# Zeudon/sound-event-localization-detection

Measured on AMD Instinct MI355X. Metric: training clips/sec (4ch FOA 60s@24kHz), higher is better.
Workload: dtype bf16; 1 GPU; crnn FOA 4-ch 60s clips, bs=32 windows (BASELINE configs[1]); parallelism=dp1

## Files before the change

include/seld_hip.h:

```cpp
#ifndef SELD_HIP_H_
#define SELD_HIP_H_

#include <stdint.h>

#ifdef __cplusplus
extern "C" {
#endif

int seld_init(int device);
int seld_shutdown(void);
int seld_version(void);
const char* seld_last_error(void);

int seld_set_mel_filterbank(const float* fb_host);

int seld_set_window(const float* window_host);

int seld_default_tables(float* window960, float* fb481x64, int* mel_b0_64, float* mel_wd_24x64,
                        float* mel_wu_24x64);

int64_t seld_num_frames(int64_t L);

int seld_logmel_f32(const float* pcm, int64_t N, int64_t C, int64_t L, float* out, int layout, void* stream);
int seld_logmel_i16(const int16_t* pcm, int64_t N, int64_t C, int64_t L, float* out, int layout, void* stream);
// ... 100 lines not shown
int64_t seld_softmax_mse_workspace_bytes(void);
int seld_softmax_mse(const void* logits, int logits_is_bf16, const uint16_t* mask, const float* dense_labels,
                     int64_t n_cells, int num_classes, float grad_scale, float* loss_out, void* grad,
                     void* workspace, void* stream);

int64_t seld_softmax_ce_workspace_bytes(void);
int seld_softmax_ce(const void* logits, int logits_is_bf16, const uint16_t* mask, const float* dense_labels,
                    int64_t n_cells, int num_classes, const float* class_weights, float focal_gamma, float grad_scale,
                    float* out, void* grad, void* workspace, void* stream);

int seld_scale_by_device_scalar(void* data, int is_bf16, int64_t n, const float* scale, void* stream);

int seld_multi_adam(const void* const* grad, const int32_t* grad_is_bf16, float* const* param, float* const* exp_avg,
                    float* const* exp_avg_sq, void* const* low_bf16, const int64_t* lengths, int count, const float* lr,
                    const float* step, float beta1, float beta2, float eps, float weight_decay, float grad_scale,
                    void* stream);

typedef struct seld_guard_record {
  float grad_norm;
  float clip_coef;
  float apply;
  float skipped;
  int32_t steps_skipped;
  int32_t steps_clipped;
  int32_t reserved[2];
} seld_guard_record;

int seld_multi_grad_norm_scratch(const int64_t* lengths, int count, int64_t* partial_floats);
int seld_multi_grad_norm(const void* const* grad, const int32_t* grad_is_bf16, const int64_t* lengths, int count,
                         float grad_scale, float max_norm, int skip_nonfinite, float* partial, int64_t partial_floats,
                         seld_guard_record* guard, void* stream);

int seld_multi_adam_guarded(const void* const* grad, const int32_t* grad_is_bf16, float* const* param,
                            float* const* exp_avg, float* const* exp_avg_sq, void* const* low_bf16, const int64_t* lengths,
                            int count, const float* lr, const float* step, float beta1, float beta2, float eps,
                            float weight_decay, float grad_scale, float* const* ema, float ema_decay,
                            const seld_guard_record* guard, void* stream);

int seld_multi_cast(const void* const* src, void* const* dst, const int64_t* lengths, int count, int bf16_to_fp32,
                    void* stream);

int seld_layernorm_supported(int64_t D);
int64_t seld_layernorm_workspace_floats(int64_t rows, int64_t D);
int seld_layernorm_forward(const void* x, int is_bf16, int64_t rows, int64_t D, const float* weight, const float* bias,
                           float eps, int relu, void* y, float* mean_rstd, void* stream);
int seld_layernorm_backward(const void* x, const void* dy, int is_bf16, int64_t rows, int64_t D, const float* weight,
                            const float* bias, const float* mean_rstd, int relu, void* dx, float* dweight,
                            float* dbias, float* workspace, void* stream);

int seld_stream_delay(int64_t nanoseconds, void* stream);

int64_t seld_smr_loss_workspace_bytes(int64_t frames, int64_t cells_per_frame);
int seld_smr_loss(const void* logits, int logits_is_bf16, const uint16_t* mask, const float* dense_labels,
                  int64_t frames, int rows, int cols, int num_classes, float w_class, float w_aiur, float w_cl,
                  float* loss_out4, void* grad, void* workspace, void* stream);


int seld_gru_fold_bias(const float* b_ih, const float* b_hh, int64_t H, void* gi_bias, int out_is_bf16, float* b_hn,
                       void* stream);

int seld_gru_prepare(const float* b_ih, const float* b_hh, const void* w_hh, int w_is_bf16, int64_t H, void* gi_bias,
                     int out_is_bf16, float* b_hn, void* w_hh_t_bf16, void* stream);

int seld_gru_bias_grads(const float* partial, int64_t tiles, int64_t H, float* db_ih, float* db_hh, void* stream);

int seld_sum_chunks(const void* partial, int in_is_bf16, int64_t chunks, int64_t count, void* out, int out_is_bf16,
                    void* stream);

int seld_sum_chunks_columns(const void* partial, int in_is_bf16, int64_t chunks, int64_t rows, int64_t C, int64_t F,
                            void* out, int out_is_bf16, void* stream);

int64_t seld_column_sums_blocks(int64_t rows, int64_t n_cols);
int seld_column_sums(const void* g, int in_is_bf16, int64_t rows, int64_t n_cols, float* partial, void* out, int out_is_bf16,
                     void* stream);

int seld_multi_sum_chunks(const void* const* partial, void* const* out, const int64_t* counts, const int32_t* chunks,
                          const int32_t* flags, int count, void* stream);
int seld_multi_column_sums_scratch(const int64_t* rows, const int64_t* n_cols, int count, int64_t* partial_floats);
int seld_multi_column_sums(const void* const* g, void* const* out, const int64_t* rows, const int64_t* n_cols,
                           const int32_t* flags, int count, float* partial, int64_t partial_floats, void* stream);

int seld_gru_dwhh_finish(const void* p_gi, const void* p_n, int in_is_bf16, int64_t chunks, int64_t H, void* dw_hh,
                         int out_is_bf16, void* stream);

int seld_conv_weight_flip_transpose(const void* w, int elem_bytes, int64_t O, int64_t I, void* wt, void* stream);

int seld_conv3x3_wgrad_supported(int64_t F, int64_t Cin, int64_t Cout);
int64_t seld_conv3x3_wgrad_workspace_floats(int64_t B, int64_t T, int64_t F, int64_t Cin, int64_t Cout);
int seld_conv3x3_wgrad(const void* x, const void* dy, int64_t B, int64_t T, int64_t F, int64_t Cin, int64_t Cout,
                       void* dw, int dw_is_bf16, float* workspace, void* stream);

int seld_conv3x3_dgrad_supported(int64_t F, int64_t Cin, int64_t Cout);
int seld_conv3x3_dgrad(const void* dy, const void* w, int64_t B, int64_t T, int64_t F, int64_t Cin, int64_t Cout,
                       void* dx, void* stream);

int seld_conv3x3_forward_supported(int64_t F, int64_t Cin, int64_t Cout);
int64_t seld_conv3x3_forward_chunks(int64_t B, int64_t T, int64_t F);
int seld_conv3x3_forward(const void* x, const void* w, int64_t B, int64_t T, int64_t F, int64_t Cin, int64_t Cout,
                         void* y, float* partials, void* stream);

int seld_convfirst_supported(int64_t F, int64_t Cin, int64_t Cout);
int64_t seld_convfirst_workspace_floats(int backward);
int seld_convfirst_forward(const void* in, const void* w, int w_is_bf16, int64_t w_sco, int64_t w_sci, int64_t w_sr,
                           int64_t w_ss, int64_t B, int64_t T, int64_t F, const float* bn_weight, const float* bn_bias,
                           float* running_mean, float* running_var, float momentum, float eps, void* y,
                           float* mean_invstd, float* scale_shift, float* workspace, int phases, void* stream);
int seld_convfirst_backward(const void* in, const void* w, int w_is_bf16, int64_t w_sco, int64_t w_sci, int64_t w_sr,
                            int64_t w_ss, const void* dy, int64_t B, int64_t T, int64_t F, const float* mean_invstd,
                            const float* scale_shift, void* dw, int dw_is_bf16, int64_t dw_sco, int64_t dw_sci,
                            int64_t dw_sr, int64_t dw_ss, float* dgamma, float* dbeta, float* workspace, int phases,
                            void* stream);

int64_t seld_conv_tail_workspace_floats(int C);
int seld_conv_tail_forward(const void* x, const void* residual, int is_bf16, int64_t rows, int C, int pool,
                           const float* weight, const float* bias, float* running_mean, float* running_var,
                           float momentum, float eps, int training, void* y, float* mean_invstd, float* scale_shift,
                           float* workspace, void* stream);
int64_t seld_conv_tail_partial_rows(void);
int seld_conv_tail_forward_from_partials(const void* x, int is_bf16, int64_t rows, int C, int pool,
                                         const float* partials, int64_t nrows, const float* weight, const float* bias,
                                         float* running_mean, float* running_var, float momentum, float eps, void* y,
                                         float* mean_invstd, float* scale_shift, void* stream);
int seld_conv_tail_backward(const void* x, const void* residual, const void* dy, int is_bf16, int64_t rows, int C,
                            int pool, const float* mean_invstd, const float* scale_shift, void* dx, void* dresidual,
                            float* dweight, float* dbias, float* workspace, void* stream);

int seld_dwconv1d(const void* x, int is_bf16, const float* weight, const float* bias, int64_t B, int64_t T, int D, int K,
                  int flip_taps, void* y, void* stream);
int64_t seld_dwconv1d_wgrad_rows(int64_t B, int64_t T);
int seld_dwconv1d_wgrad(const void* x, const void* dy, int is_bf16, int64_t B, int64_t T, int D, int K, float* partial,
                        void* stream);

int64_t seld_gru_tile_rows(void);
int seld_gru_forward(const void* gi, int is_bf16, const void* w_hh_bf16, const float* b_hn, int64_t B,
                     int64_t T, int64_t H, void* y, void* saved_tile, void* stream);

int seld_gru_backward(const void* dy_tile, const void* saved_tile, const void* y, int is_bf16,
                      const void* w_hh_t_bf16, int64_t tiles, int64_t T, int64_t H, void* dg_tile, float* dbias,
                      void* stream);

int seld_gru_backward_direct(const void* dy, const void* saved_tile, const void* y, int is_bf16,
                             const void* w_hh_t_bf16, int64_t B, int64_t T, int64_t H, void* dgi, void* dghn,
                             float* dbias, void* stream);

int seld_gru_to_tile(const void* src, int elem_bytes, int64_t B, int64_t T, int ns, void* dst, void* stream);
int seld_gru_from_pair_tile(const void* dg_tile, int elem_bytes, int64_t B, int64_t T, void* dgi, void* dghn,
                            void* stream);

int seld_gru_previous_state(const void* y, int elem_bytes, int64_t B, int64_t T, void* h_prev, void* stream);

int seld_grid_decode(const void* logits, int is_bf16, int64_t w0, int64_t nw, int64_t W, int64_t total,
                     const int64_t* meta_first, const int32_t* meta_len, int64_t q0, int64_t nq, float threshold, int K,
                     int32_t* det_cell, float* det_score, int32_t* det_count, float* probs_out, void* stream);

int seld_doa_match(const int32_t* det_cell, const int32_t* det_count, int K, const int32_t* ref_offsets,
                   const int32_t* ref_dirs, int64_t nq, int I, int J, double thr_deg, int32_t* stats, double* cost,
                   void* stream);

int seld_grid_decode_tta(const void* logits, int is_bf16, int64_t w0, int64_t nw, int64_t W, int64_t total,
                         const int64_t* meta_first, const int32_t* meta_len, int64_t q0, int64_t nq,
                         const int32_t* patterns, int n_patterns, float threshold, int K, int32_t* det_cell,
                         float* det_score, int32_t* det_count, float* probs_out, void* stream);

int seld_track_link(const int32_t* det_cell, const int32_t* det_count, int K, const int64_t* seg_offsets, int64_t S,
                    const int32_t* dist_table, int I, int J, int gate_mdeg, int max_gap, int min_len,
                    const int64_t* chain_offsets, int32_t* trk_cell, int32_t* trk_id, int32_t* trk_count, int32_t* tracks,
// ... 44 lines not shown
```

sound-event-localization-detection_amd/seld_gru.py:

```python
import torch
import torch.nn.functional as F

import seld_native
import seld_overlap
from seld_linear import chunk_count, tall_chunks, tall_product

HIDDEN = 256
direct_backward = True


def applicable(module, x):
    low = torch.is_autocast_enabled() or x.dtype in (torch.bfloat16, torch.float16)
    if not low and not getattr(module, "allow_fp32", False):
        return False
    return (module.hidden_size == HIDDEN and module.bidirectional and module.batch_first and module.bias
            and x.dim() == 3 and x.dtype in (torch.float32, torch.bfloat16, torch.float16) and module.proj_size == 0)


class _BiGRULayer(torch.autograd.Function):
    @staticmethod
    def forward(ctx, x, w_ih, b_ih, w_hh, b_hh, overlap=False, feature_cf=None):
        ctx.overlap = overlap
        ctx.feature_cf = feature_cf
        if feature_cf is not None:
            c, f = feature_cf
            w_ih = w_ih.view(w_ih.shape[0], c, f).transpose(1, 2).reshape(w_ih.shape[0], f * c)
        low = torch.is_autocast_enabled() or x.dtype == torch.bfloat16
        cdt = torch.bfloat16 if low else torch.float32
        with torch.autocast(device_type="cuda", enabled=False):
            xc = x.to(cdt)
            need = x.requires_grad or w_ih.requires_grad or w_hh.requires_grad
            w_hh_t = None
            if b_ih.dtype == torch.float32 and b_hh.dtype == torch.float32 and b_ih.is_contiguous() and b_hh.is_contiguous():
                if (direct_backward and need and w_hh.is_contiguous()
                        and w_hh.dtype in (torch.float32, torch.bfloat16)):
                    gi_bias, b_hn, w_hh_t = seld_native.gru_prepare(b_ih, b_hh.reshape(-1), w_hh, cdt)
                else:
                    gi_bias, b_hn = seld_native.gru_fold_bias(b_ih, b_hh.reshape(-1), cdt)
            else:
                fold = b_hh.clone()
                fold[:, 2 * HIDDEN:] = 0
                gi_bias, b_hn = (b_ih + fold.reshape(-1)).to(cdt), b_hh[:, 2 * HIDDEN:]
            gi = F.linear(xc, w_ih.to(cdt), gi_bias)
            b, t, _ = gi.shape
            y, saved = seld_native.gru_forward(gi.view(b, t, 2, 3 * HIDDEN), w_hh, b_hn, need)
        ctx.save_for_backward(xc, w_ih, w_hh, y, saved if saved is not None else torch.empty(0),
                              w_hh_t if w_hh_t is not None else torch.empty(0))
        ctx.cdt = cdt
        ctx.dtypes = (w_ih.dtype, b_ih.dtype, w_hh.dtype, b_hh.dtype)
        return y

    @staticmethod
    def backward(ctx, dy):
        xc, w_ih, w_hh, y, saved, w_hh_t = ctx.saved_tensors
        cdt = ctx.cdt
        b, t, _ = y.shape
        h = HIDDEN
        n = b * t
        with torch.autocast(device_type="cuda", enabled=False):
            dyc = dy.to(y.dtype)
            seld_overlap.launch_pending(dy.device)
            dgi, dghn, dbias = seld_native.gru_backward(dyc, saved, y, w_hh, raw_bias=True,
                                                        w_hh_t=w_hh_t if w_hh_t.numel() else None, direct=direct_backward)
            dgi2 = dgi.view(n, 6 * h)
            x2 = xc.reshape(n, -1)
            t_wih, t_bih, t_whh, t_bhh = ctx.dtypes

            dw_ih = torch.empty((6 * h, x2.shape[1]), dtype=t_wih, device=dy.device)
            dw_hh = torch.empty((2, 3 * h, h), dtype=t_whh, device=dy.device)
            db_ih = torch.empty(6 * h, dtype=t_bih, device=dy.device)
            db_hh = torch.empty(6 * h, dtype=t_bhh, device=dy.device)

            def weight_grads():
                fp32 = [db if db.dtype == torch.float32 else torch.empty(6 * h, dtype=torch.float32, device=dy.device)
                        for db in (db_ih, db_hh)]
                seld_native.gru_bias_grads(dbias, out=fp32)
                for db, full in zip((db_ih, db_hh), fp32):
                    if db is not full:
                        db.copy_(full)
                tall_product(dgi2, x2, out=dw_ih, columns_cf=ctx.feature_cf)
                hp = seld_native.gru_previous_state(y).view(n, 2 * h)
                chunks = chunk_count(n, 6 * h, 2 * h)
                p_gi = tall_chunks(dgi2, hp, chunks)
                p_n = tall_chunks(dghn.view(n, 2 * h), hp, chunks)
                seld_native.gru_dwhh_finish(p_gi, p_n, dw_hh)

            dx = (dgi2 @ w_ih.to(cdt)).view_as(xc)
            if ctx.overlap:
                seld_overlap.submit(dy.device, [dgi, dghn, y, xc, dbias, dw_ih, dw_hh, db_ih, db_hh], weight_grads)
            elif seld_overlap.conv_wgrad_side and seld_overlap.enabled and dy.is_cuda:
                seld_overlap.launch_now(dy.device, [dgi, dghn, y, xc, dbias, dw_ih, dw_hh, db_ih, db_hh], weight_grads,
                                        last_of_stage=True, outputs=[dw_ih, dw_hh, db_ih, db_hh])
            else:
                weight_grads()
        return dx.to(dy.dtype) if dx.dtype != dy.dtype and not torch.is_autocast_enabled() else dx, \
            dw_ih.view_as(dw_ih), db_ih.view_as(db_ih), dw_hh.view_as(dw_hh), db_hh.view(2, 3 * h), None, None


from seld_pack import adjacent as _adjacent, join as _join, pack as _pack


def pack_parameters(module):
    with torch.no_grad():
        for layer in range(module.num_layers):
            for kind in ("weight_ih", "bias_ih", "weight_hh", "bias_hh"):
                _pack((getattr(module, f"{kind}_l{layer}"), getattr(module, f"{kind}_l{layer}_reverse")))


def bigru_forward(module, x, feature_cf=None, overlap=False, need_hn=True):
    overlap = overlap and seld_overlap.active(x)
    params = []
    for layer in range(module.num_layers):
        p = lambda name: getattr(module, f"{name}_l{layer}")
        pr = lambda name: getattr(module, f"{name}_l{layer}_reverse")
        group = (_join(p("weight_ih"), pr("weight_ih")), _join(p("bias_ih"), pr("bias_ih")),
                 _join(p("weight_hh"), pr("weight_hh")), _join(p("bias_hh"), pr("bias_hh")))
        params.append(seld_overlap.defer(*group) if overlap and layer > 0 else group)
    out = x
    finals = []
    for layer in range(module.num_layers):
        w_ih, b_ih, w_hh, b_hh = params[layer]
        out = _BiGRULayer.apply(out, w_ih, b_ih, w_hh.view(2, 3 * HIDDEN, HIDDEN), b_hh.view(2, 3 * HIDDEN),
                                overlap and layer > 0, feature_cf if layer == 0 else None)
        if need_hn:
            finals += [out[:, -1, :HIDDEN], out[:, 0, HIDDEN:]]
        if module.training and module.dropout > 0 and layer + 1 < module.num_layers:
            out = F.dropout(out, p=module.dropout, training=True)
    return out, (torch.stack(finals, dim=0) if need_hn else None)
```

sound-event-localization-detection_amd/seld_native.py:

```python
from __future__ import annotations

import ctypes
import os
import threading
from pathlib import Path

import torch

from seld_augment import PARAM_INTS as AUGMENT_PARAM_INTS, PATTERNS as AUGMENT_PATTERNS, check_channel_order

_HERE = Path(__file__).resolve().parent
LIB_PATH = Path(os.environ["SELD_HIP_LIB"]).resolve() if os.environ.get("SELD_HIP_LIB") else _HERE / "libseld_hip.so"

N_FFT = 960
HOP = 480
N_BINS = 481
N_MELS = 64

_lock = threading.Lock()
_lib = None
_initialised_devices = set()

_i64 = ctypes.c_int64
_int = ctypes.c_int
# ... 15 lines not shown
    lib.seld_default_tables.argtypes = [_ptr] * 5
    lib.seld_num_frames.restype = _i64
    lib.seld_num_frames.argtypes = [_i64]
    for name in ("seld_logmel_f32", "seld_logmel_i16"):
        getattr(lib, name).argtypes = [_ptr, _i64, _i64, _i64, _ptr, _int, _ptr]
    for name in ("seld_logmel_f32_strided", "seld_logmel_i16_strided"):
        getattr(lib, name).argtypes = [_ptr, _i64, _i64, _i64, _ptr, _i64, _i64, _i64, _i64, _ptr]
    for name in ("seld_stft_f32", "seld_stft_i16"):
        getattr(lib, name).argtypes = [_ptr, _i64, _i64, _i64, _ptr, _ptr]
    lib.seld_foa_intensity.argtypes = [_ptr, _i64, _i64, _ptr, _i64, _i64, _i64, _i64, _ptr]
    for fn in (lib.seld_logmel_iv_f32, lib.seld_logmel_iv_i16):
        fn.argtypes = [_ptr, _i64, _i64, _ptr, _i64, _i64, _i64, _i64, _ptr]
    for fn in (lib.seld_logmel_spectrum_f32, lib.seld_logmel_spectrum_i16):
        fn.argtypes = [_ptr, _i64, _i64, _i64, _ptr, _i64, _i64, _i64, _i64, _ptr, _ptr]
        fn.restype = ctypes.c_int
    for fn in (lib.seld_logmel_phasors_f32, lib.seld_logmel_phasors_i16):
        fn.argtypes = [_ptr, _i64, _i64, _i64, _ptr, _i64, _i64, _i64, _i64, _ptr, _ptr]
    lib.seld_phasor_pitch.restype = ctypes.c_int64
    lib.seld_gcc_phat_q15.argtypes = [_ptr, _i64, _i64, _i64, _ptr, _i64, _i64, _i64, _i64, _ptr]
    lib.seld_gcc_table_host.argtypes = [_ptr]
    lib.seld_gcc_phat.argtypes = [_ptr, _i64, _i64, _i64, _ptr, _i64, _i64, _i64, _i64, _ptr]
    lib.seld_nipd_table_host.argtypes = [ctypes.c_double, ctypes.c_double, ctypes.c_double, _ptr, _ptr, _ptr, _ptr]
    lib.seld_nipd_table_bytes.restype = _i64
    lib.seld_nipd_table_bytes.argtypes = []
    lib.seld_nipd_q15.argtypes = [_ptr, _i64, _i64, _i64, _ptr, _ptr, _i64, _i64, _i64, _i64, _ptr]
    lib.seld_labels_rasterise.argtypes = [_ptr, _i64, _i64, _int, _int, _ptr, _ptr]
    lib.seld_labels_expand.argtypes = [_ptr, _i64, _int, _ptr, _ptr]
    lib.seld_labels_rasterise_box.argtypes = [_ptr, _ptr, _i64, _i64, _int, _int, ctypes.c_double, ctypes.c_double, _ptr,
                                              _ptr]
    lib.seld_window_gather.argtypes = [_ptr, _i64, _i64, _ptr, _i64, _i64, _ptr, _ptr]
    lib.seld_window_gather_augment.argtypes = [_ptr, _i64, _int, _int, _ptr, _ptr, _i64, _i64, _ptr, ctypes.c_float, _ptr, _ptr]
    lib.seld_window_permute_mask.argtypes = [_ptr, _i64, _int, _int, _ptr, _ptr, _i64, _i64, _ptr, _ptr]
    lib.seld_foa_rotation_terms.argtypes = [_ptr, _i64, _i64, _int, _int, _ptr, _i64, _i64, _i64, _i64, _ptr]
    lib.seld_window_gather_rotate.argtypes = [_ptr, _ptr, _i64, _int, _int, _int, _int, _int, _int, _ptr, _ptr, _i64, _i64, _ptr,
                                              ctypes.c_float, _ptr, _ptr]
    lib.seld_window_permute_mask_rotate.argtypes = [_ptr, _i64, _int, _int, _ptr, _ptr, _i64, _i64, _ptr, _ptr]
    lib.seld_feature_moments_workspace.restype = _i64
    lib.seld_feature_moments_workspace.argtypes = [_i64, _int]
    lib.seld_feature_moments.argtypes = [_ptr, _i64, _int, _ptr, _ptr, _i64, _ptr]
    lib.seld_window_gather_affine.argtypes = [_ptr, _i64, _int, _ptr, _i64, _i64, _ptr, _ptr, _ptr, _ptr]
    lib.seld_window_gather_augment_affine.argtypes = [_ptr, _i64, _int, _int, _ptr, _ptr, _i64, _i64, _ptr, ctypes.c_float,
                                                      _ptr, _ptr, _ptr, _ptr]
    lib.seld_window_gather_rotate_affine.argtypes = [_ptr, _ptr, _i64, _int, _int, _int, _int, _int, _int, _ptr, _ptr, _i64,
                                                     _i64, _ptr, ctypes.c_float, _ptr, _ptr, _ptr, _ptr]
    lib.seld_window_gather_mix.argtypes = [_ptr, _i64, _int, _int, _ptr, _ptr, _ptr, _i64, _i64, _ptr, ctypes.c_float, _int,
                                           _ptr, _ptr]
    lib.seld_window_gather_mix_standardised.argtypes = [_ptr, _i64, _int, _int, _ptr, _ptr, _ptr, _i64, _i64, _ptr, ctypes.c_float,
                                                  _int, _ptr, _ptr, _ptr, _ptr]
    lib.seld_window_mix_mask.argtypes = [_ptr, _i64, _int, _int, _ptr, _ptr, _ptr, _i64, _i64, _ptr, _ptr]
    lib.seld_softmax_mse_workspace_bytes.restype = _i64
    lib.seld_softmax_mse_workspace_bytes.argtypes = []
    lib.seld_softmax_mse.argtypes = [_ptr, _int, _ptr, _ptr, _i64, _int, ctypes.c_float, _ptr, _ptr, _ptr, _ptr]
    lib.seld_softmax_ce_workspace_bytes.restype = _i64
    lib.seld_softmax_ce_workspace_bytes.argtypes = []
    lib.seld_softmax_ce.argtypes = [_ptr, _int, _ptr, _ptr, _i64, _int, _ptr, ctypes.c_float, ctypes.c_float, _ptr, _ptr,
                                    _ptr, _ptr]
    lib.seld_scale_by_device_scalar.argtypes = [_ptr, _int, _i64, _ptr, _ptr]
    lib.seld_smr_loss_workspace_bytes.restype = _i64
    lib.seld_smr_loss_workspace_bytes.argtypes = [_i64, _i64]
    lib.seld_smr_loss.argtypes = [_ptr, _int, _ptr, _ptr, _i64, _int, _int, _int, ctypes.c_float, ctypes.c_float,
                                  ctypes.c_float, _ptr, _ptr, _ptr, _ptr]
    lib.seld_multi_cast.argtypes = [_ptr, _ptr, _ptr, _int, _int, _ptr]
    lib.seld_stream_delay.argtypes = [_i64, _ptr]
    lib.seld_gru_fold_bias.argtypes = [_ptr, _ptr, _i64, _ptr, _int, _ptr, _ptr]
    lib.seld_gru_prepare.argtypes = [_ptr, _ptr, _ptr, _int, _i64, _ptr, _int, _ptr, _ptr, _ptr]
    lib.seld_gru_bias_grads.argtypes = [_ptr, _i64, _i64, _ptr, _ptr, _ptr]
    lib.seld_sum_chunks.argtypes = [_ptr, _int, _i64, _i64, _ptr, _int, _ptr]
    lib.seld_sum_chunks_columns.argtypes = [_ptr, _int, _i64, _i64, _i64, _i64, _ptr, _int, _ptr]
    lib.seld_gru_dwhh_finish.argtypes = [_ptr, _ptr, _int, _i64, _i64, _ptr, _int, _ptr]
    lib.seld_column_sums.argtypes = [_ptr, _int, _i64, _i64, _ptr, _ptr, _int, _ptr]
    _pp, _pi64, _pi32 = ctypes.POINTER(ctypes.c_void_p), ctypes.POINTER(ctypes.c_int64), ctypes.POINTER(ctypes.c_int32)
    _f = ctypes.c_float
    lib.seld_multi_adam.argtypes = [_pp, _pi32, _pp, _pp, _pp, _pp, _pi64, _int, _ptr, _ptr, _f, _f, _f, _f, _f, _ptr]
    lib.seld_multi_grad_norm_scratch.argtypes = [_pi64, _int, _pi64]
    lib.seld_multi_grad_norm.argtypes = [_pp, _pi32, _pi64, _int, _f, _f, _int, _ptr, _i64, _ptr, _ptr]
    lib.seld_multi_adam_guarded.argtypes = [_pp, _pi32, _pp, _pp, _pp, _pp, _pi64, _int, _ptr, _ptr, _f, _f, _f, _f, _f, _pp, _f,
                                            _ptr, _ptr]
    lib.seld_multi_sum_chunks.argtypes = [_pp, _pp, _pi64, _pi32, _pi32, _int, _ptr]
    lib.seld_multi_column_sums_scratch.argtypes = [_pi64, _pi64, _int, _pi64]
    lib.seld_multi_column_sums.argtypes = [_pp, _pp, _pi64, _pi64, _pi32, _int, _ptr, _i64, _ptr]
    lib.seld_column_sums_blocks.argtypes = [_i64, _i64]
    lib.seld_column_sums_blocks.restype = ctypes.c_int64
    lib.seld_conv_weight_flip_transpose.argtypes = [_ptr, _int, _i64, _i64, _ptr, _ptr]
    lib.seld_conv3x3_wgrad_supported.argtypes = [_i64, _i64, _i64]
    lib.seld_conv3x3_wgrad_workspace_floats.restype = _i64
    lib.seld_conv3x3_wgrad_workspace_floats.argtypes = [_i64, _i64, _i64, _i64, _i64]
    lib.seld_conv3x3_wgrad.argtypes = [_ptr, _ptr, _i64, _i64, _i64, _i64, _i64, _ptr, _int, _ptr, _ptr]
    lib.seld_conv3x3_dgrad_supported.argtypes = [_i64, _i64, _i64]
    lib.seld_conv3x3_dgrad.argtypes = [_ptr, _ptr, _i64, _i64, _i64, _i64, _i64, _ptr, _ptr]
    lib.seld_conv3x3_forward_supported.argtypes = [_i64, _i64, _i64]
    lib.seld_conv3x3_forward_chunks.restype = _i64
    lib.seld_conv3x3_forward_chunks.argtypes = [_i64, _i64, _i64]
    lib.seld_conv3x3_forward.argtypes = [_ptr, _ptr, _i64, _i64, _i64, _i64, _i64, _ptr, _ptr, _ptr]
    lib.seld_conv_tail_partial_rows.restype = _i64
    lib.seld_conv_tail_partial_rows.argtypes = []
    lib.seld_conv_tail_forward_from_partials.argtypes = [_ptr, _int, _i64, _int, _int, _ptr, _i64, _ptr, _ptr, _ptr, _ptr,
                                                         ctypes.c_float, ctypes.c_float, _ptr, _ptr, _ptr, _ptr]
    lib.seld_convfirst_supported.argtypes = [_i64, _i64, _i64]
    lib.seld_convfirst_workspace_floats.restype = _i64
    lib.seld_convfirst_workspace_floats.argtypes = [_int]
    lib.seld_convfirst_forward.argtypes = [_ptr, _ptr, _int, _i64, _i64, _i64, _i64, _i64, _i64, _i64, _ptr, _ptr, _ptr, _ptr,
                                           ctypes.c_float, ctypes.c_float, _ptr, _ptr, _ptr, _ptr, _int, _ptr]
    lib.seld_convfirst_backward.argtypes = [_ptr, _ptr, _int, _i64, _i64, _i64, _i64, _ptr, _i64, _i64, _i64, _ptr, _ptr,
                                            _ptr, _int, _i64, _i64, _i64, _i64, _ptr, _ptr, _ptr, _int, _ptr]
    lib.seld_layernorm_supported.argtypes = [_i64]
    lib.seld_layernorm_workspace_floats.restype = _i64
    lib.seld_layernorm_workspace_floats.argtypes = [_i64, _i64]
    lib.seld_layernorm_forward.argtypes = [_ptr, _int, _i64, _i64, _ptr, _ptr, ctypes.c_float, _int, _ptr, _ptr, _ptr]
    lib.seld_layernorm_backward.argtypes = [_ptr, _ptr, _int, _i64, _i64, _ptr, _ptr, _ptr, _int, _ptr, _ptr, _ptr,
                                            _ptr, _ptr]
    lib.seld_conv_tail_workspace_floats.restype = _i64
    lib.seld_conv_tail_workspace_floats.argtypes = [_int]
    lib.seld_conv_tail_forward.argtypes = [_ptr, _ptr, _int, _i64, _int, _int, _ptr, _ptr, _ptr, _ptr, ctypes.c_float,
                                           ctypes.c_float, _int, _ptr, _ptr, _ptr, _ptr, _ptr]
    lib.seld_conv_tail_backward.argtypes = [_ptr, _ptr, _ptr, _int, _i64, _int, _int, _ptr, _ptr, _ptr, _ptr, _ptr, _ptr,
                                            _ptr, _ptr]
    lib.seld_dwconv1d.argtypes = [_ptr, _int, _ptr, _ptr, _i64, _i64, _int, _int, _int, _ptr, _ptr]
    lib.seld_dwconv1d_wgrad.argtypes = [_ptr, _ptr, _int, _i64, _i64, _int, _int, _ptr, _ptr]
    lib.seld_dwconv1d_wgrad_rows.argtypes = [_i64, _i64]
    lib.seld_dwconv1d_wgrad_rows.restype = ctypes.c_int64
    lib.seld_gru_to_tile.argtypes = [_ptr, _int, _i64, _i64, _int, _ptr, _ptr]
    lib.seld_gru_from_pair_tile.argtypes = [_ptr, _int, _i64, _i64, _ptr, _ptr, _ptr]
    lib.seld_gru_previous_state.argtypes = [_ptr, _int, _i64, _i64, _ptr, _ptr]
    lib.seld_gru_tile_rows.restype = _i64
    lib.seld_gru_tile_rows.argtypes = []
    lib.seld_gru_forward.argtypes = [_ptr, _int, _ptr, _ptr, _i64, _i64, _i64, _ptr, _ptr, _ptr]
    lib.seld_gru_backward.argtypes = [_ptr, _ptr, _ptr, _int, _ptr, _i64, _i64, _i64, _ptr, _ptr, _ptr]
    lib.seld_gru_backward_direct.argtypes = [_ptr, _ptr, _ptr, _int, _ptr, _i64, _i64, _i64, _ptr, _ptr, _ptr, _ptr]
    lib.seld_grid_decode.argtypes = [_ptr, _int, _i64, _i64, _i64, _i64, _ptr, _ptr, _i64, _i64, ctypes.c_float, _int,
                                     _ptr, _ptr, _ptr, _ptr, _ptr]
    lib.seld_doa_match.argtypes = [_ptr, _ptr, _int, _ptr, _ptr, _i64, _int, _int, ctypes.c_double, _ptr, _ptr, _ptr]
    lib.seld_grid_decode_tta.argtypes = [_ptr, _int, _i64, _i64, _i64, _i64, _ptr, _ptr, _i64, _i64, _pi32, _int,
                                         ctypes.c_float, _int, _ptr, _ptr, _ptr, _ptr, _ptr]
    lib.seld_track_link.argtypes = [_ptr, _ptr, _int, _ptr, _i64, _ptr, _int, _int, _int, _int, _int, _ptr, _ptr, _ptr, _ptr,
                                    _ptr, _ptr, _ptr]
    lib.seld_grid_decode_refine.argtypes = [_ptr, _int, _i64, _i64, _i64, _i64, _ptr, _ptr, _i64, _i64, _pi32, _int,
                                            ctypes.c_float, _int, _ptr, _ptr, _ptr, _ptr, _ptr, _ptr, _ptr]
    lib.seld_doa_match_dirs.argtypes = [_ptr, _ptr, _int, _ptr, _ptr, _i64, ctypes.c_double, _ptr, _ptr, _ptr]
    lib.seld_doa_match_prefix.argtypes = [_ptr, _ptr, _ptr, _int, _ptr, _ptr, _i64, _int, _int, ctypes.c_double, _ptr, _ptr,
                                          _ptr]
    lib.seld_sweep_score.argtypes = [_ptr, _ptr, _ptr, _ptr, _int, _ptr, _i64, ctypes.POINTER(ctypes.c_float), _int, _i64,
                                     _ptr, _ptr, _ptr, _ptr]
    lib.seld_doa_assign.argtypes = [_ptr, _ptr, _ptr, _int, _ptr, _ptr, _i64, _int, _int, ctypes.c_double, _ptr, _ptr]
    lib.seld_segment_score.argtypes = [_ptr, _ptr, _int, _ptr, _ptr, _ptr, _i64, ctypes.c_double, _ptr, _ptr, _ptr, _ptr,
                                       _ptr, _ptr]
    lib.seld_jackknife_score.argtypes = [_ptr, _ptr, _ptr, _i64, _ptr, _ptr, _ptr]
    lib.seld_resample_plan.argtypes =[_i64, _i64, _pi32, _pi32, _pi32, _pi32]
    lib.seld_resample_table_host.argtypes = [_i64, _i64, _ptr, _ptr]
    for fn in (lib.seld_resample_f32, lib.seld_resample_i16):
        fn.argtypes = [_ptr, _i64, _i64, _i64, _ptr, _int, _int, _int, _int, _ptr, _i64, _ptr]
    return lib


def load_library():
    global _lib
    if _lib is not None:
        return _lib
    with _lock:
        if _lib is None:
            if not LIB_PATH.exists():
                raise SeldNativeError(
                    f"{LIB_PATH} not found: build it with `python -c 'import __graft_entry__ as g; g.build()'` "
                    f"or `make -C {_HERE / 'csrc'}`.  There is no CPU fallback.")
            lib = _declare(ctypes.CDLL(str(LIB_PATH)))
            global GRU_TILE
            GRU_TILE = int(lib.seld_gru_tile_rows())
# ... 1206 lines not shown

def column_sums(g: torch.Tensor, out: torch.Tensor) -> torch.Tensor:
    if not column_sums_supported(g, out):
        raise SeldNativeError("column_sums: g [rows, N] contiguous bf16 / fp32 with N % 8 == 0, out [N] contiguous")
    lib = load_library()
    rows, n = g.shape
    blocks = int(lib.seld_column_sums_blocks(rows, n))
    partial = torch.empty((blocks, n), dtype=torch.float32, device=g.device)
    with _device_guard(ensure_init(g.device)):
        check(lib.seld_column_sums(_p(g), _is_bf16(g), rows, n, _p(partial), _p(out), _is_bf16(out), _stream_ptr(g.device)),
              "seld_column_sums")
    return out


def multi_sum_chunks(pairs) -> None:
    pairs = list(pairs)
    if not pairs:
        return
    for partial, out in pairs:
        if not (partial.is_cuda and partial.is_contiguous() and out.is_contiguous()
                and tuple(partial.shape[1:]) == tuple(out.shape) and partial.dtype in (torch.float32, torch.bfloat16)
                and out.dtype in (torch.float32, torch.bfloat16)):
            raise SeldNativeError("multi_sum_chunks: partial [chunks, ...] / out [...] contiguous bf16 or fp32")
    n = len(pairs)
    src = (ctypes.c_void_p * n)(*[p.data_ptr() for p, _ in pairs])
    dst = (ctypes.c_void_p * n)(*[o.data_ptr() for _, o in pairs])
    counts = (ctypes.c_int64 * n)(*[o.numel() for _, o in pairs])
    chunks = (ctypes.c_int32 * n)(*[p.shape[0] for p, _ in pairs])
    flags = (ctypes.c_int32 * n)(*[_is_bf16(p) | (_is_bf16(o) << 1) for p, o in pairs])
    device = pairs[0][1].device
    with _device_guard(ensure_init(device)):
        check(load_library().seld_multi_sum_chunks(src, dst, counts, chunks, flags, n, _stream_ptr(device)),
              "seld_multi_sum_chunks")


_column_scratch = {}
_retired_scratch = []


def multi_column_sums(pairs) -> None:
    pairs = list(pairs)
    if not pairs:
        return
    for g, out in pairs:
        if not column_sums_supported(g, out):
            raise SeldNativeError("multi_column_sums: g [rows, N] contiguous bf16 / fp32 with N % 8 == 0, out [N] contiguous")
    lib = load_library()
    n = len(pairs)
    src = (ctypes.c_void_p * n)(*[g.data_ptr() for g, _ in pairs])
    dst = (ctypes.c_void_p * n)(*[o.data_ptr() for _, o in pairs])
    rows = (ctypes.c_int64 * n)(*[g.shape[0] for g, _ in pairs])
    cols = (ctypes.c_int64 * n)(*[g.shape[1] for g, _ in pairs])
    flags = (ctypes.c_int32 * n)(*[_is_bf16(g) | (_is_bf16(o) << 1) for g, o in pairs])
    need_f = ctypes.c_int64(0)
    check(lib.seld_multi_column_sums_scratch(rows, cols, n, ctypes.byref(need_f)), "seld_multi_column_sums_scratch")
    device = pairs[0][0].device
    index = ensure_init(device)
    scratch = _column_scratch.get(index)
    if scratch is None or scratch.numel() < need_f.value:
        if torch.cuda.is_current_stream_capturing():
            raise SeldNativeError("multi_column_sums: the scratch must be sized by an eager call before a graph capture")
        if scratch is not None:
            _retired_scratch.append(scratch)
        scratch = torch.empty(max(need_f.value, 1 << 20), dtype=torch.float32, device=device)
        _column_scratch[index] = scratch
    with _device_guard(index):
        check(lib.seld_multi_column_sums(src, dst, rows, cols, flags, n, _p(scratch), scratch.numel(), _stream_ptr(device)),
              "seld_multi_column_sums")


def gru_dwhh_finish(p_gi: torch.Tensor, p_n: torch.Tensor, out: torch.Tensor) -> torch.Tensor:
    chunks = p_gi.shape[0]
    h = out.shape[2]
    if not (p_gi.is_contiguous() and p_n.is_contiguous() and out.is_contiguous() and p_gi.dtype == p_n.dtype
            and tuple(p_gi.shape) == (chunks, 6 * h, 2 * h) and tuple(p_n.shape) == (chunks, 2 * h, 2 * h)
            and tuple(out.shape) == (2, 3 * h, h)):
        raise SeldNativeError("gru_dwhh_finish: shapes must be [chunks, 6H, 2H], [chunks, 2H, 2H] -> [2, 3H, H]")
    with _device_guard(ensure_init(out.device)):
        check(load_library().seld_gru_dwhh_finish(_p(p_gi), _p(p_n), _is_bf16(p_gi), chunks, h, _p(out), _is_bf16(out),
                                                  _stream_ptr(out.device)), "seld_gru_dwhh_finish")
    return out


def conv_weight_flip_transpose(w: torch.Tensor) -> torch.Tensor:
    o, i, kh, kw = w.shape
    if not (w.is_cuda and kh == 3 and kw == 3 and w.dtype in (torch.float32, torch.bfloat16)
            and w.is_contiguous(memory_format=torch.channels_last)):
        raise SeldNativeError("conv_weight_flip_transpose: 3x3 weights in channels-last memory expected")
    wt = torch.empty((i, o, 3, 3), dtype=w.dtype, device=w.device, memory_format=torch.channels_last)
    with _device_guard(ensure_init(w.device)):
        check(load_library().seld_conv_weight_flip_transpose(_p(w), w.element_size(), o, i, _p(wt),
                                                             _stream_ptr(w.device)), "seld_conv_weight_flip_transpose")
    return wt


def conv3x3_wgrad_applicable(x: torch.Tensor, dy: torch.Tensor, w: torch.Tensor) -> bool:
    if not (x.is_cuda and x.dim() == 4 and dy.dim() == 4 and w.dim() == 4 and x.dtype == torch.bfloat16
            and dy.dtype == torch.bfloat16 and tuple(w.shape[2:]) == (3, 3)):
        return False
    b, cin, t, f = x.shape
    if tuple(dy.shape) != (b, w.shape[0], t, f) or w.shape[1] != cin:
        return False
    if not (x.is_contiguous(memory_format=torch.channels_last) and dy.is_contiguous(memory_format=torch.channels_last)
            and w.is_contiguous(memory_format=torch.channels_last)):
        return False
    return bool(load_library().seld_conv3x3_wgrad_supported(f, cin, w.shape[0]))


def conv3x3_wgrad(x: torch.Tensor, dy: torch.Tensor, dw: torch.Tensor) -> torch.Tensor:
    if not conv3x3_wgrad_applicable(x, dy, dw) or dw.dtype not in (torch.float32, torch.bfloat16):
        raise SeldNativeError("conv3x3_wgrad: unsupported shapes, dtypes or layouts")
    b, cin, t, f = x.shape
    cout = dy.shape[1]
    with _device_guard(ensure_init(x.device)):
        lib = load_library()
        ws = torch.empty(int(lib.seld_conv3x3_wgrad_workspace_floats(b, t, f, cin, cout)), dtype=torch.float32,
                         device=x.device)
        check(lib.seld_conv3x3_wgrad(_p(x), _p(dy), b, t, f, cin, cout, _p(dw), _is_bf16(dw), _p(ws),
                                     _stream_ptr(x.device)), "seld_conv3x3_wgrad")
    return dw


def conv3x3_dgrad_applicable(dy: torch.Tensor, w: torch.Tensor) -> bool:
    if not (dy.is_cuda and dy.dim() == 4 and w.dim() == 4 and dy.dtype == torch.bfloat16 and w.dtype == torch.bfloat16
            and tuple(w.shape[2:]) == (3, 3) and dy.shape[1] == w.shape[0]):
        return False
    if not (dy.is_contiguous(memory_format=torch.channels_last) and w.is_contiguous(memory_format=torch.channels_last)):
        return False
    return bool(load_library().seld_conv3x3_dgrad_supported(dy.shape[3], w.shape[1], w.shape[0]))


def conv3x3_dgrad(dy: torch.Tensor, w: torch.Tensor, out: "torch.Tensor | None" = None) -> torch.Tensor:
    if not conv3x3_dgrad_applicable(dy, w):
        raise SeldNativeError("conv3x3_dgrad: unsupported shapes, dtypes or layouts")
    b, cout, t, f = dy.shape
    cin = w.shape[1]
    if out is None:
        out = torch.empty((b, cin, t, f), dtype=torch.bfloat16, device=dy.device, memory_format=torch.channels_last)
    elif not (out.dtype == torch.bfloat16 and out.device == dy.device and tuple(out.shape) == (b, cin, t, f)
              and out.is_contiguous(memory_format=torch.channels_last)):
        raise SeldNativeError("conv3x3_dgrad: out must be bf16 [B, Cin, T, F] in channels-last memory")
    with _device_guard(ensure_init(dy.device)):
        check(load_library().seld_conv3x3_dgrad(_p(dy), _p(w), b, t, f, cin, cout, _p(out), _stream_ptr(dy.device)),
              "seld_conv3x3_dgrad")
    return out


def conv3x3_forward_applicable(x: torch.Tensor, w: torch.Tensor) -> bool:
    if not (x.is_cuda and x.dim() == 4 and w.dim() == 4 and x.dtype == torch.bfloat16 and w.dtype == torch.bfloat16
            and tuple(w.shape[2:]) == (3, 3) and x.shape[1] == w.shape[1]):
        return False
    if not (x.is_contiguous(memory_format=torch.channels_last) and w.is_contiguous(memory_format=torch.channels_last)):
        return False
    return bool(load_library().seld_conv3x3_forward_supported(x.shape[3], w.shape[1], w.shape[0]))


def conv3x3_forward_supported(f: int, cin: int, cout: int) -> bool:
    return bool(load_library().seld_conv3x3_forward_supported(f, cin, cout))


def conv_tail_partial_rows() -> int:
    return int(load_library().seld_conv_tail_partial_rows())


def conv3x3_forward_chunks(b: int, t: int, f: int) -> int:
    return int(load_library().seld_conv3x3_forward_chunks(b, t, f))
# ... 226 lines not shown
```

Baseline: 176.2 clips/s.

## Add fused MFMA kernel computing GRU recurrent weight gradient from shifted hidden states

Adds a dedicated HIP kernel that computes dW_hh directly from the gate gradients and the output sequence. It builds the time-shifted previous-state rows on the fly with halo and padding masking, stages tiles in double-buffered LDS, and accumulates with bf16 MFMA over batch slabs, followed by a small slab-sum kernel. This replaces the separate previous-state materialisation, chunked tall products and finish reduction. By default it is used for GRU layers after the first, or for all layers when an environment flag is set, so the first layer still takes the old path when it runs beside the conv wgrads. It adds a per-call fp32 workspace allocation and a new code path that is only valid for H=256 and bf16 inputs.

```diff
diff --git a/include/seld_hip.h b/include/seld_hip.h
--- a/include/seld_hip.h
+++ b/include/seld_hip.h
@@ -206,6 +206,10 @@
 
 int seld_gru_dwhh_finish(const void* p_gi, const void* p_n, int in_is_bf16, int64_t chunks, int64_t H, void* dw_hh,
                          int out_is_bf16, void* stream);
+
+int64_t seld_gru_dwhh_workspace_bytes(int64_t B, int64_t T);
+int seld_gru_dwhh(const void* dgi, const void* dghn, const void* y, int64_t B, int64_t T, int64_t H, void* workspace,
+                  int64_t workspace_bytes, void* dw_hh, int out_is_bf16, void* stream);
 
 int seld_conv_weight_flip_transpose(const void* w, int elem_bytes, int64_t O, int64_t I, void* wt, void* stream);
 
diff --git a/sound-event-localization-detection_amd/csrc/gru_dwhh.hip b/sound-event-localization-detection_amd/csrc/gru_dwhh.hip
--- /dev/null
+++ b/sound-event-localization-detection_amd/csrc/gru_dwhh.hip
@@ -0,0 +1,202 @@
+#include <hip/hip_bf16.h>
+
+#include "conv3x3_image.h"
+#include "gru_dwhh_rows.h"
+#include "seld_common.h"
+
+namespace seld {
+
+namespace {
+
+using namespace conv3x3;
+
+constexpr int kDwH = 256;
+constexpr int kDwThreads = 512;
+constexpr int kDwTile = 128;
+constexpr int kDwPitch = 2 * kDwTile + 16;
+constexpr int kDwImageShorts = kDwhhChunk * kDwPitch;
+constexpr int kDwSumThreads = 256;
+constexpr long kDwCount = 2L * 3 * kDwH * kDwH;
+constexpr int kDwLaunchBound = 2 * kDwThreads;
+static_assert(kDwPitch * 2 % 64 == 32, "row pitch: an odd number of 32-byte units");
+static_assert(kDwhhChunk == 64 && kDwhhChunk * 16 == 2 * kDwThreads, "two gate and two y pieces per thread and chunk");
+static_assert(2 * kDwImageShorts * 2 <= 96 * 1024, "LDS budget");
+
+struct Pieces {
+  uint4 g[2], y[2];
+};
+
+__global__ __launch_bounds__(kDwLaunchBound) void gru_dwhh_kernel(
+    const unsigned short* __restrict__ dgi, const unsigned short* __restrict__ dghn,
+    const unsigned short* __restrict__ y, int B, int T, int per_slab, float* __restrict__ ws) {
+  __shared__ __attribute__((aligned(16))) unsigned short lds[2 * kDwImageShorts];
+
+  const int mt = blockIdx.x >> 1, nt = blockIdx.x & 1, dir = blockIdx.y, slab = blockIdx.z;
+  const int gate = mt >> 1;
+  const unsigned short* const gsrc = gate < 2 ? dgi + dir * 3 * kDwH + gate * kDwH + (mt & 1) * kDwTile
+                                               : dghn + dir * kDwH + (mt & 1) * kDwTile;
+  const long gstride = gate < 2 ? 6 * kDwH : 2 * kDwH;
+  const unsigned short* const ysrc = y + dir * kDwH + nt * kDwTile;
+  const int seqs = min(per_slab, B - slab * per_slab);
+  const int chunks = (seqs * T + kDwhhChunk - 1) / kDwhhChunk;
+
+  f32x4 acc[4][2];
+#pragma unroll
+  for (int m = 0; m < 4; ++m)
+#pragma unroll
+    for (int n = 0; n < 2; ++n) acc[m][n] = f32x4{0.0f, 0.0f, 0.0f, 0.0f};
+
+  const int mod32 = 32 % T, mod64 = kDwhhChunk % T;
+  DwhhWalk w_load = dwhh_walk_begin(threadIdx.x >> 4, T), w_store = w_load;
+  auto load = [&](Pieces& r) {
+    int tid = threadIdx.x;
+    asm volatile("" : "+v"(tid));
+    const int col = (tid & 15) * 8;
+    const DwhhWalk w[2] = {w_load, dwhh_walk_step(w_load, 32, mod32, T)};
+#pragma unroll
+    for (int i = 0; i < 2; ++i) {
+      const DwhhRow row = dwhh_row(B, T, per_slab, slab, w[i], dir);
+      r.g[i] = *reinterpret_cast<const uint4*>(gsrc + row.g_row * gstride + col);
+      r.y[i] = *reinterpret_cast<const uint4*>(ysrc + row.y_row * (2 * kDwH) + col);
+    }
+    w_load = dwhh_walk_step(w_load, kDwhhChunk, mod64, T);
+  };
+  auto store = [&](unsigned short* image, const Pieces& r) {
+    int tid = threadIdx.x;
+    asm volatile("" : "+v"(tid));
+    const int col = (tid & 15) * 8;
+    auto piece_or_zero = [](uint4 v, bool keep) {
+      return make_uint4(keep ? v.x : 0u, keep ? v.y : 0u, keep ? v.z : 0u, keep ? v.w : 0u);
+    };
+    const DwhhWalk w[2] = {w_store, dwhh_walk_step(w_store, 32, mod32, T)};
+#pragma unroll
+    for (int i = 0; i < 2; ++i) {
+      const DwhhRow row = dwhh_row(B, T, per_slab, slab, w[i], dir);
+      unsigned short* const dst = image + ((tid >> 4) + 32 * i) * kDwPitch + col;
+      *reinterpret_cast<uint4*>(dst) = piece_or_zero(r.g[i], !row.padding);
+      *reinterpret_cast<uint4*>(dst + kDwTile) = piece_or_zero(r.y[i], !row.padding && !row.halo);
+    }
+    w_store = dwhh_walk_step(w_store, kDwhhChunk, mod64, T);
+  };
+  auto step = [&](int c, unsigned short* cur, unsigned short* other, Pieces& held, Pieces& next, bool inner) {
+    __syncthreads();
+    if (inner || c + 2 < chunks) load(next);
+    __builtin_amdgcn_sched_barrier(0);
+    int lt = threadIdx.x;
+    asm volatile("" : "+v"(lt));
+    const int g = (lt >> 4) & 3, q = (lt >> 2) & 3, p = lt & 3, wv = lt >> 6;
+    const unsigned short* const pa = cur + (4 * g + q) * kDwPitch + (wv >> 2) * 64 + 4 * p;
+    const unsigned short* const pb = cur + (4 * g + q) * kDwPitch + kDwTile + (wv & 3) * 32 + 4 * p;
+#pragma unroll
+    for (int ks = 0; ks < kDwhhChunk / 32; ++ks) {
+      bf16x8 a[4], b[2];
+#pragma unroll
+      for (int m = 0; m < 4; ++m)
+        a[m] = join(tr_read(pa, ks * 32 * kDwPitch + m * 16), tr_read(pa, (ks * 32 + 16) * kDwPitch + m * 16));
+#pragma unroll
+      for (int n = 0; n < 2; ++n)
+        b[n] = join(tr_read(pb, ks * 32 * kDwPitch + n * 16), tr_read(pb, (ks * 32 + 16) * kDwPitch + n * 16));
+#pragma unroll
+      for (int m = 0; m < 4; ++m)
+#pragma unroll
+        for (int n = 0; n < 2; ++n) acc[m][n] = __builtin_amdgcn_mfma_f32_16x16x32_bf16(a[m], b[n], acc[m][n], 0, 0, 0);
+    }
+    __builtin_amdgcn_sched_barrier(0);
+    if (inner || c + 1 < chunks) store(other, held);
+  };
+
+  Pieces r0, r1;
+  load(r0);
+  store(lds, r0);
+  if (chunks > 1) load(r0);
+  unsigned short* const lds1 = lds + kDwImageShorts;
+  int c = 0;
+  for (; c + 3 < chunks; c += 2) {
+    step(c, lds, lds1, r0, r1, true);
+    step(c + 1, lds1, lds, r1, r0, true);
+  }
+  step(c, lds, lds1, r0, r1, false);
+  if (c + 1 < chunks) step(c + 1, lds1, lds, r1, r0, false);
+  if (c + 2 < chunks) step(c + 2, lds, lds1, r0, r1, false);
+
+  const int lane = threadIdx.x & 63, wm = threadIdx.x >> 8, wn = (threadIdx.x >> 6) & 3;
+  float* const slot = ws + (static_cast<long>(slab) * 2 + dir) * (3 * kDwH * kDwH);
+#pragma unroll
+  for (int m = 0; m < 4; ++m)
+#pragma unroll
+    for (int j = 0; j < 4; ++j) {
+      const int row = mt * kDwTile + wm * 64 + m * 16 + 4 * (lane >> 4) + j;
+#pragma unroll
+      for (int n = 0; n < 2; ++n)
+        slot[static_cast<long>(row) * kDwH + nt * kDwTile + wn * 32 + n * 16 + (lane & 15)] = acc[m][n][j];
+    }
+}
+
+template <bool kBf16>
+__global__ __launch_bounds__(kDwSumThreads) void gru_dwhh_sum_kernel(const float* __restrict__ ws, int slabs,
+                                                                      void* __restrict__ dw) {
+  const long i = (static_cast<long>(blockIdx.x) * kDwSumThreads + threadIdx.x) * 4;
+  if (i >= kDwCount) return;
+  float4 s = *reinterpret_cast<const float4*>(ws + i);
+  for (int k = 1; k < slabs; ++k) {
+    const float4 v = *reinterpret_cast<const float4*>(ws + k * kDwCount + i);
+    s.x += v.x; s.y += v.y; s.z += v.z; s.w += v.w;
+  }
+  if (kBf16) {
+    const unsigned lo = static_cast<unsigned>(__bfloat16_as_ushort(__float2bfloat16(s.x))) |
+                        (static_cast<unsigned>(__bfloat16_as_ushort(__float2bfloat16(s.y))) << 16);
+    const unsigned hi = static_cast<unsigned>(__bfloat16_as_ushort(__float2bfloat16(s.z))) |
+                        (static_cast<unsigned>(__bfloat16_as_ushort(__float2bfloat16(s.w))) << 16);
+    *reinterpret_cast<uint2*>(static_cast<unsigned short*>(dw) + i) = make_uint2(lo, hi);
+  } else {
+    *reinterpret_cast<float4*>(static_cast<float*>(dw) + i) = s;
+  }
+}
+
+bool dwhh_shape_ok(int64_t B, int64_t T, int64_t H) {
+  return H == kDwH && B > 0 && T > 0 && B <= (1 << 20) && T <= (1 << 20) && B * T <= (1LL << 30);
+}
+
+}
+
+}
+
+extern "C" {
+
+int64_t seld_gru_dwhh_workspace_bytes(int64_t B, int64_t T) {
+  using namespace seld;
+  if (!dwhh_shape_ok(B, T, kDwH)) return 0;
+  return static_cast<int64_t>(dwhh_plan(B, T).slabs) * kDwCount * static_cast<int64_t>(sizeof(float));
+}
+
+int seld_gru_dwhh(const void* dgi, const void* dghn, const void* y, int64_t B, int64_t T, int64_t H, void* workspace,
+                  int64_t workspace_bytes, void* dw_hh, int out_is_bf16, void* stream_) {
+  using namespace seld;
+  const DeviceState* st = current_state();
+  if (!st) return kErrNotInitialised;
+  if (!dgi || !dghn || !y || !workspace || !dw_hh) return fail(kErrInvalidArgument, "seld_gru_dwhh: null argument");
+  if (H != kDwH) return fail(kErrUnsupported, "seld_gru_dwhh: H must be 256");
+  if (!dwhh_shape_ok(B, T, H)) return fail(kErrInvalidArgument, "seld_gru_dwhh: B, T must be positive, B * T <= 2^30");
+  if (((reinterpret_cast<uintptr_t>(dgi) | reinterpret_cast<uintptr_t>(dghn) | reinterpret_cast<uintptr_t>(y) |
+        reinterpret_cast<uintptr_t>(workspace) | reinterpret_cast<uintptr_t>(dw_hh)) & 15) != 0)
+    return fail(kErrInvalidArgument, "seld_gru_dwhh: 16-byte aligned tensors required");
+  if (workspace_bytes < seld_gru_dwhh_workspace_bytes(B, T))
+    return fail(kErrInvalidArgument, "seld_gru_dwhh: workspace smaller than seld_gru_dwhh_workspace_bytes");
+  const DwhhPlan pl = dwhh_plan(B, T);
+  hipStream_t stream = static_cast<hipStream_t>(stream_);
+  float* const ws = static_cast<float*>(workspace);
+  const dim3 grid(3 * kDwH / kDwTile * (kDwH / kDwTile), 2, static_cast<unsigned>(pl.slabs));
+  hipLaunchKernelGGL(gru_dwhh_kernel, grid, dim3(kDwThreads), 0, stream, static_cast<const unsigned short*>(dgi),
+                     static_cast<const unsigned short*>(dghn), static_cast<const unsigned short*>(y),
+                     static_cast<int>(B), static_cast<int>(T), pl.per_slab, ws);
+  SELD_HIP_TRY(hipGetLastError());
+  const dim3 sum_grid(static_cast<unsigned>((kDwCount / 4 + kDwSumThreads - 1) / kDwSumThreads));
+  if (out_is_bf16)
+    hipLaunchKernelGGL(gru_dwhh_sum_kernel<true>, sum_grid, dim3(kDwSumThreads), 0, stream, ws, pl.slabs, dw_hh);
+  else
+    hipLaunchKernelGGL(gru_dwhh_sum_kernel<false>, sum_grid, dim3(kDwSumThreads), 0, stream, ws, pl.slabs, dw_hh);
+  SELD_HIP_TRY(hipGetLastError());
+  return kOk;
+}
+
+}
diff --git a/sound-event-localization-detection_amd/csrc/gru_dwhh_rows.h b/sound-event-localization-detection_amd/csrc/gru_dwhh_rows.h
--- /dev/null
+++ b/sound-event-localization-detection_amd/csrc/gru_dwhh_rows.h
@@ -0,0 +1,70 @@
+#pragma once
+
+#if defined(__HIPCC__) || defined(__CUDACC__)
+#define SELD_DWHH_HD __host__ __device__ inline
+#else
+#define SELD_DWHH_HD inline
+#endif
+
+namespace seld {
+
+constexpr int kDwhhChunk = 64;
+constexpr int kDwhhMaxSlabs = 8;
+
+struct DwhhPlan {
+  int per_slab;
+  int slabs;
+  int chunks;
+};
+
+SELD_DWHH_HD DwhhPlan dwhh_plan(long B, long T) {
+  DwhhPlan pl;
+  const long want = B < kDwhhMaxSlabs ? B : kDwhhMaxSlabs;
+  pl.per_slab = static_cast<int>((B + want - 1) / want);
+  pl.slabs = static_cast<int>((B + pl.per_slab - 1) / pl.per_slab);
+  pl.chunks = static_cast<int>((pl.per_slab * T + kDwhhChunk - 1) / kDwhhChunk);
+  return pl;
+}
+
+struct DwhhRow {
+  long g_row;
+  long y_row;
+  bool padding;
+  bool halo;
+};
+
+struct DwhhWalk {
+  int row;
+  int t;
+};
+
+SELD_DWHH_HD DwhhWalk dwhh_walk_begin(int row, int T) {
+  DwhhWalk w;
+  w.row = row;
+  w.t = row % T;
+  return w;
+}
+
+SELD_DWHH_HD DwhhWalk dwhh_walk_step(DwhhWalk w, int step, int step_mod, int T) {
+  const int t = w.t + step_mod;
+  w.row += step;
+  w.t = t >= T ? t - T : t;
+  return w;
+}
+
+SELD_DWHH_HD DwhhRow dwhh_row(int B, int T, int per_slab, int slab, DwhhWalk w, int dir) {
+  const int seq0 = slab * per_slab;
+  const int seqs = B - seq0 < per_slab ? B - seq0 : per_slab;
+  const long first = static_cast<long>(seq0) * T;
+  const int edge = dir == 0 ? 0 : T - 1, shift = dir == 0 ? -1 : 1;
+  DwhhRow r;
+  r.padding = w.row >= seqs * T;
+  r.halo = !r.padding & (w.t == edge);
+  const int g_local = r.padding ? 0 : w.row;
+  const int y_local = g_local + ((r.padding | r.halo) ? 0 : shift);
+  r.g_row = first + g_local;
+  r.y_row = first + y_local;
+  return r;
+}
+
+}
diff --git a/sound-event-localization-detection_amd/seld_gru.py b/sound-event-localization-detection_amd/seld_gru.py
--- a/sound-event-localization-detection_amd/seld_gru.py
+++ b/sound-event-localization-detection_amd/seld_gru.py
@@ -1,3 +1,5 @@
+import os
+
 import torch
 import torch.nn.functional as F
 
@@ -7,6 +9,8 @@
 
 HIDDEN = 256
 direct_backward = True
+own_dwhh = True
+own_dwhh_beside_convs = os.environ.get("SELD_OWN_DWHH_BESIDE_CONVS", "0") == "1"
 
 
 def applicable(module, x):
@@ -19,8 +23,9 @@
 
 class _BiGRULayer(torch.autograd.Function):
     @staticmethod
-    def forward(ctx, x, w_ih, b_ih, w_hh, b_hh, overlap=False, feature_cf=None):
+    def forward(ctx, x, w_ih, b_ih, w_hh, b_hh, overlap=False, feature_cf=None, first_layer=False):
         ctx.overlap = overlap
+        ctx.first_layer = first_layer
         ctx.feature_cf = feature_cf
         if feature_cf is not None:
             c, f = feature_cf
@@ -71,6 +76,9 @@
             db_ih = torch.empty(6 * h, dtype=t_bih, device=dy.device)
             db_hh = torch.empty(6 * h, dtype=t_bhh, device=dy.device)
 
+            beside_convs = not ctx.overlap and seld_overlap.conv_wgrad_side and seld_overlap.enabled and dy.is_cuda
+            use_own_dwhh = own_dwhh and (own_dwhh_beside_convs or not ctx.first_layer)
+
             def weight_grads():
                 fp32 = [db if db.dtype == torch.float32 else torch.empty(6 * h, dtype=torch.float32, device=dy.device)
                         for db in (db_ih, db_hh)]
@@ -79,6 +87,9 @@
                     if db is not full:
                         db.copy_(full)
                 tall_product(dgi2, x2, out=dw_ih, columns_cf=ctx.feature_cf)
+                if use_own_dwhh and seld_native.GRU_TILE == 4 and seld_native.gru_dwhh_supported(dgi, dghn, y, dw_hh):
+                    seld_native.gru_dwhh(dgi, dghn, y, dw_hh)
+                    return
                 hp = seld_native.gru_previous_state(y).view(n, 2 * h)
                 chunks = chunk_count(n, 6 * h, 2 * h)
                 p_gi = tall_chunks(dgi2, hp, chunks)
@@ -88,13 +99,13 @@
             dx = (dgi2 @ w_ih.to(cdt)).view_as(xc)
             if ctx.overlap:
                 seld_overlap.submit(dy.device, [dgi, dghn, y, xc, dbias, dw_ih, dw_hh, db_ih, db_hh], weight_grads)
-            elif seld_overlap.conv_wgrad_side and seld_overlap.enabled and dy.is_cuda:
+            elif beside_convs:
                 seld_overlap.launch_now(dy.device, [dgi, dghn, y, xc, dbias, dw_ih, dw_hh, db_ih, db_hh], weight_grads,
                                         last_of_stage=True, outputs=[dw_ih, dw_hh, db_ih, db_hh])
             else:
                 weight_grads()
         return dx.to(dy.dtype) if dx.dtype != dy.dtype and not torch.is_autocast_enabled() else dx, \
-            dw_ih.view_as(dw_ih), db_ih.view_as(db_ih), dw_hh.view_as(dw_hh), db_hh.view(2, 3 * h), None, None
+            dw_ih.view_as(dw_ih), db_ih.view_as(db_ih), dw_hh.view_as(dw_hh), db_hh.view(2, 3 * h), None, None, None
 
 
 from seld_pack import adjacent as _adjacent, join as _join, pack as _pack
@@ -121,7 +132,7 @@
     for layer in range(module.num_layers):
         w_ih, b_ih, w_hh, b_hh = params[layer]
         out = _BiGRULayer.apply(out, w_ih, b_ih, w_hh.view(2, 3 * HIDDEN, HIDDEN), b_hh.view(2, 3 * HIDDEN),
-                                overlap and layer > 0, feature_cf if layer == 0 else None)
+                                overlap and layer > 0, feature_cf if layer == 0 else None, layer == 0)
         if need_hn:
             finals += [out[:, -1, :HIDDEN], out[:, 0, HIDDEN:]]
         if module.training and module.dropout > 0 and layer + 1 < module.num_layers:
diff --git a/sound-event-localization-detection_amd/seld_native.py b/sound-event-localization-detection_amd/seld_native.py
--- a/sound-event-localization-detection_amd/seld_native.py
+++ b/sound-event-localization-detection_amd/seld_native.py
@@ -121,6 +121,9 @@
     lib.seld_column_sums_blocks.argtypes = [_i64, _i64]
     lib.seld_column_sums_blocks.restype = ctypes.c_int64
     lib.seld_conv_weight_flip_transpose.argtypes = [_ptr, _int, _i64, _i64, _ptr, _ptr]
+    lib.seld_gru_dwhh_workspace_bytes.restype = _i64
+    lib.seld_gru_dwhh_workspace_bytes.argtypes = [_i64, _i64]
+    lib.seld_gru_dwhh.argtypes = [_ptr, _ptr, _ptr, _i64, _i64, _i64, _ptr, _i64, _ptr, _int, _ptr]
     lib.seld_conv3x3_wgrad_supported.argtypes = [_i64, _i64, _i64]
     lib.seld_conv3x3_wgrad_workspace_floats.restype = _i64
     lib.seld_conv3x3_wgrad_workspace_floats.argtypes = [_i64, _i64, _i64, _i64, _i64]
@@ -1493,6 +1496,29 @@
     return out
 
 
+def gru_dwhh_supported(dgi: torch.Tensor, dghn: torch.Tensor, y: torch.Tensor, out: torch.Tensor) -> bool:
+    if not (dgi.is_cuda and dgi.dim() == 5 and dgi.dtype == dghn.dtype == y.dtype == torch.bfloat16):
+        return False
+    b, t, h = dgi.shape[0], dgi.shape[1], GRU_H
+    if b < 1 or t < 1 or b * t > 1 << 30:
+        return False
+    return (tuple(dgi.shape) == (b, t, 2, 3, h) and tuple(dghn.shape) == (b, t, 2, h) and tuple(y.shape) == (b, t, 2 * h)
+            and tuple(out.shape) == (2, 3 * h, h) and out.dtype in (torch.float32, torch.bfloat16)
+            and all(x.is_contiguous() and x.data_ptr() % 16 == 0 and x.device == dgi.device for x in (dgi, dghn, y, out)))
+
+
+def gru_dwhh(dgi: torch.Tensor, dghn: torch.Tensor, y: torch.Tensor, out: torch.Tensor) -> torch.Tensor:
+    if not gru_dwhh_supported(dgi, dghn, y, out):
+        raise SeldNativeError("gru_dwhh: unsupported shapes, dtypes or layouts")
+    b, t = dgi.shape[0], dgi.shape[1]
+    with _device_guard(ensure_init(dgi.device)):
+        lib = load_library()
+        ws = torch.empty(int(lib.seld_gru_dwhh_workspace_bytes(b, t)), dtype=torch.uint8, device=dgi.device)
+        check(lib.seld_gru_dwhh(_p(dgi), _p(dghn), _p(y), b, t, GRU_H, _p(ws), ws.numel(), _p(out), _is_bf16(out),
+                                _stream_ptr(dgi.device)), "seld_gru_dwhh")
+    return out
+
+
 def conv_weight_flip_transpose(w: torch.Tensor) -> torch.Tensor:
     o, i, kh, kw = w.shape
     if not (w.is_cuda and kh == 3 and kw == 3 and w.dtype in (torch.float32, torch.bfloat16)
```

Result: no change. 176.1 clips/s (median of 2 runs) (-0.0%).
